# TUI-NICR/EMSANet

Hardware: AMD Instinct MI355X
Metric: images/sec (640x480 RGB-D, bs=32/GPU) fwd+bwd (higher is better)
Workload: dtype f32; 1 GPU; BASELINE.json configs[1]: full EMSANet RGB-D (resnet34-NBt1D x2, SE-add fusion, PPM, semantic+instance+orientation+scene heads), 640x480, bs=32/GPU, f32, train mode (BN batch stats, Dropout2d), step = fwd + bwd (fixed output cotangents) + grad all-reduce + SGD-nesterov update at lr 0 (fixed weights) replayed from a hipGraph; global_batch=32, parallelism=dp1, weights=random init (deterministic), mode=train-hipgraph

## Files before the change

### emsanet_amd/_lib.py

```python
import ctypes
import os
from ctypes import POINTER, Structure, c_char_p, c_float, c_int, c_int8, c_int32, c_int64, c_uint32, c_void_p

LIB_PATH = os.environ.get('EMSA_LIB') or os.path.join(
    os.path.dirname(os.path.abspath(__file__)), 'lib', 'libemsanet_hip.so')


class EmsaPackJob(Structure):
    _fields_ = [('src', c_void_p), ('dst0', c_void_p), ('dst1', c_void_p), ('cout', c_int32),
                ('cin', c_int32), ('kh', c_int32), ('kw', c_int32), ('kind', c_int32),
                ('first_block', c_int32), ('cout_total', c_int32), ('cout_off', c_int32),
                ('cin_total', c_int32), ('cin_off', c_int32)]


PACK_GEMM = 0
PACK_WINO = 1
PACK_GEMM_16 = {1: 2, 2: 3}
PACK_COPY = 4
PACK_FRAG_16 = {1: 5, 2: 6}
PACK_WINO2D = 7


class EmsaDropoutJob(Structure):
    _fields_ = [('offset', c_int64), ('c', c_int32), ('layer_id', c_uint32), ('p', c_float),
# ... 12 lines not shown
        ('in_img_stride', c_int64), ('in_row_stride', c_int64),
        ('in_px_stride', c_int32), ('ld_out', c_int32),
        ('out_pix_img', c_int32), ('out_pix_row', c_int32), ('out_pix_px', c_int32),
        ('out_pix_off', c_int32),
    ]


class EmsaTargetScale(Structure):
    _fields_ = [('scale', c_int32), ('sigma', c_int32), ('semantic', c_void_p), ('center', c_void_p),
                ('offset', c_void_p), ('foreground', c_void_p), ('orientation', c_void_p),
                ('orientation_foreground', c_void_p)]


class EmsaExportJob(Structure):
    _fields_ = [('src0', c_void_p), ('src1', c_void_p), ('depth', c_void_p), ('lut', c_void_p),
                ('dst', c_void_p), ('divisor', c_int64), ('max_depth', ctypes.c_double),
                ('kind', c_int32), ('src0_dtype', c_int32), ('src1_dtype', c_int32),
                ('depth_dtype', c_int32), ('lut_size', c_int32), ('add', c_int32), ('h', c_int32),
                ('w', c_int32)]


class EmsaNormalScale(Structure):
    _fields_ = [('scale', c_int32), ('reserved', c_int32), ('out', c_void_p)]


_P = c_void_p
_GP = POINTER(EmsaConvGeom)
_TP = POINTER(EmsaTargetScale)

SIGNATURES = {
    'emsa_arch': (c_char_p, []),
    'emsa_version': (c_int, []),
    'emsa_set_batch_invariant': (c_int, [c_int]),
    'emsa_conv_igemm': (c_int, [_GP, _P, _P, _P, _P, _P, _P, _P, _P, c_int32, _P, c_int32, c_int32, _P]),
    'emsa_conv_stats_rows': (c_int, [_GP]),
    'emsa_conv1d_wino_supported': (c_int, [_GP]),
    'emsa_conv1d_wino_stats_rows': (c_int, [_GP]),
    'emsa_conv_relu_bits_words': (c_int64, [c_int64, c_int32]),
    'emsa_conv1d_wino_bnb': (c_int, [_GP, _P, _P, _P, _P, c_int32, _P, c_int32, _P, _P, _P, _P, _P,
                                     c_int32, _P]),
    'emsa_conv_igemm_bnb_t': (c_int, [c_int32, _GP, _P, _P, _P, _P, c_int32, _P, c_int32, _P, _P, _P, _P,
                                      _P, c_int32, _P]),
    'emsa_bn_bwd_apply_rows_t': (c_int, [c_int32, _P, _P, _P, _P, _P, _P, c_int32, c_int32, c_int64,
                                         c_int32, c_int32, _P, _P, _P, _P]),
    'emsa_conv1d_wino': (c_int, [_GP, _P, _P, _P, _P, _P, _P, _P, _P, c_int32, _P, c_int32, c_int32, _P,
                                 _P, _P]),
    'emsa_memset_async': (c_int, [_P, c_int32, c_int64, _P]),
    'emsa_graph_count_nodes': (c_int, [_P, POINTER(c_int32), POINTER(c_int32), POINTER(c_int32)]),
    'emsa_graph_replace_memsets': (c_int, [_P, POINTER(c_int32)]),
    'emsa_dropout2d_mask_batch': (c_int, [_P, _P, c_int32, c_int32, c_int32, c_uint32, _P, _P]),
    'emsa_to_nhwc_t': (c_int, [c_int32, _P, _P, c_int32, c_int32, c_int32, c_int32, c_int64, c_int64,
                               c_int64, c_int64, _P]),
    'emsa_conv1d_wino_set_spec': (c_int, [c_int32]),
    'emsa_conv1d_wino_spec_launches': (c_int, []),
    'emsa_conv1d_wino_resmask_supported': (c_int, [_GP, c_int32]),
    'emsa_conv1d_wino_resmask': (c_int, [_GP, _P, _P, _P, _P, c_int32, _P, _P]),
    'emsa_bn_act_fwd_wbits': (c_int, [_P, _P, _P, _P, _P, _P, c_int32, c_int64, c_int32, c_int32, _P, _P]),
    'emsa_bn_act_fwd_raff': (c_int, [_P] * 8 + [c_int32, c_int64, c_int32, c_int32, _P, c_int32, _P]),
    'emsa_bn_bwd_reduce_wbits': (c_int, [_P, _P, _P, _P, _P, _P, c_int32, c_int64, c_int32, _P, _P]),
    'emsa_bn_bwd_apply_wbits': (c_int, [_P] * 8 + [c_int32, c_int32, c_int64, c_int32, c_int32] + [_P] * 5),
    'emsa_conv1d_wino_inbn': (c_int, [_GP, _P, _P, _P, _P, _P, _P, _P, c_int32, _P, _P]),
    'emsa_conv_wgrad_inbn': (c_int, [_GP, _P, _P, _P, _P, _P, _P, _P, _P]),
    'emsa_conv_wgrad_inbn_t': (c_int, [c_int32, _GP, _P, _P, _P, _P, _P, _P, _P, _P]),
    'emsa_conv_wgrad_multi_inbn_t': (c_int, [c_int32, c_int32, _GP, POINTER(c_void_p), POINTER(c_void_p),
                                             POINTER(c_void_p), POINTER(c_void_p), _P,
                                             POINTER(c_void_p), POINTER(c_void_p), _P]),
    'emsa_conv1d_rs_inbn_t': (c_int, [c_int32, _GP, _P, _P, _P, _P, _P, _P, _P, c_int32, _P]),
    'emsa_bn_bwd_reduce_aff_t': (c_int, [c_int32, _P, _P, _P, _P, _P, _P, c_int32, c_int64, c_int32, _P, _P]),
    'emsa_bn_bwd_apply_aff_t': (c_int, [c_int32, _P, _P, _P, _P, _P, _P, _P, _P, c_int32, c_int32, c_int64,
                                        c_int32, _P, _P, _P, _P]),
    'emsa_conv_wgrad_multi_ws_bytes': (c_int64, [c_int32, c_int32, _GP]),
    'emsa_conv_wgrad_multi_t': (c_int, [c_int32, c_int32, _GP, POINTER(c_void_p), POINTER(c_void_p),
                                        POINTER(c_void_p), POINTER(c_void_p), _P, _P]),
    'emsa_pack_wino': (c_int, [_P, _P, _P, c_int32, c_int32, c_int32, _P]),
    'emsa_pack_batch': (c_int, [_P, c_int32, c_int32, _P]),
    'emsa_conv_wino2d_supported': (c_int, [_GP]),
    'emsa_conv_wino2d_stats_rows': (c_int, [_GP]),
    'emsa_conv_wino2d': (c_int, [_GP, _P, _P, _P, _P, _P, _P, _P, _P, c_int32, _P, c_int32, c_int32, _P]),
    'emsa_conv_wgrad_wino2d_supported': (c_int, [c_int32, _GP]),
    'emsa_conv_wgrad_wino2d_ws_bytes': (c_int64, [c_int32, _GP]),
    'emsa_conv_wgrad_wino2d_split_steps': (c_int, [c_int32, _GP]),
    'emsa_conv_wgrad_wino2d': (c_int, [c_int32, _GP, _P, _P, _P, _P, _P, c_int32, _P]),
    'emsa_pack_wino2d': (c_int, [_P, _P, _P, c_int32, c_int32, _P]),
    'emsa_pack_wino2d_packed': (c_int, [_P, _P, c_int32, c_int32, c_int32, _P]),
    'emsa_pack_wino_packed': (c_int, [_P, _P, c_int32, c_int32, c_int32, c_int32, _P]),
    'emsa_conv_wgrad_ws_bytes': (c_int64, [_GP]),
    'emsa_conv_wgrad': (c_int, [_GP, _P, _P, _P, _P, _P, _P]),
    'emsa_pack_weight_fwd': (c_int, [_P, _P] + [c_int32] * 8 + [_P]),
    'emsa_pack_weight_dgrad': (c_int, [_P, _P] + [c_int32] * 8 + [_P]),
    'emsa_unpack_wgrad': (c_int, [_P, _P] + [c_int32] * 8 + [_P]),
    'emsa_pack_weight_pair': (c_int, [_P, _P, _P] + [c_int32] * 4 + [_P]),
    'emsa_stem_pack_input': (c_int, [_P, _P, c_int32, c_int32, c_int32, c_int32, _P]),
    'emsa_stem_pack_weight': (c_int, [_P, _P, c_int32, c_int32, _P]),
    'emsa_stem_pack_input_rows_t': (c_int, [c_int32, _P, _P, c_int32, c_int32, c_int32, _P]),
    'emsa_stem_pack_weight_rows_t': (c_int, [c_int32, _P, _P, c_int32, _P]),
    'emsa_stem_unpack_wgrad_rows': (c_int, [_P, _P, c_int32, _P]),
    'emsa_stem_unpack_wgrad': (c_int, [_P, _P, c_int32, c_int32, _P]),
    'emsa_bn_finalize': (c_int, [_P, c_int32, c_int32, c_int64, _P, _P, c_float, c_float,
                                 _P, _P, _P, _P, _P, _P, _P, _P]),
    'emsa_bn_finalize_ws_bytes': (c_int, [c_int32]),
    'emsa_bn_fold': (c_int, [_P, _P, _P, _P, c_float, c_int32, _P, _P, _P, _P]),
    'emsa_relu_mask_words': (c_int64, [c_int64]),
    'emsa_bn_act_fwd': (c_int, [_P, _P, _P, _P, _P, _P, c_int32, c_int64, c_int32, c_int32, _P,
                                _P]),
    'emsa_bn_bwd_reduce': (c_int, [_P, _P, _P, _P, _P, _P, _P, c_int32, c_int64, c_int32, c_int32,
                                   _P, _P]),
# ... 216 lines not shown
```

### emsanet_amd/csrc/common.h

```cpp
#pragma once
#include <hip/hip_runtime.h>
#include <stdint.h>

#include "emsanet_hip.h"

typedef float f32x16 __attribute__((ext_vector_type(16)));
typedef float f32x4 __attribute__((ext_vector_type(4)));

#define EMSA_WAVE 64
#define EMSA_NXCD 8

static inline int emsa_launch_status() {
  return hipGetLastError() == hipSuccess ? EMSA_OK : EMSA_E_LAUNCH;
}

__device__ __forceinline__ int emsa_xcd_remap(int bid, int nwg) {
  const int q = nwg / EMSA_NXCD, r = nwg % EMSA_NXCD;
  const int xcd = bid % EMSA_NXCD, idx = bid / EMSA_NXCD;
  const int base = xcd < r ? xcd * (q + 1) : r * (q + 1) + (xcd - r) * q;
  return base + idx;
}

__device__ __forceinline__ float4 emsa_ld4(const float* p) {
  return *reinterpret_cast<const float4*>(p);
}
__device__ __forceinline__ void emsa_st4(float* p, float4 v) {
  *reinterpret_cast<float4*>(p) = v;
}
__device__ __forceinline__ float4 emsa_zero4() { return make_float4(0.f, 0.f, 0.f, 0.f); }

__host__ __device__ __forceinline__ size_t emsa_wino2d_at(int comp, int n, int k, int n_ch, int k_ch) {
  return ((((size_t)comp * ((k_ch + 7) >> 3) + (k >> 3)) * n_ch + n) << 3) + (k & 7);
}
__host__ __device__ __forceinline__ int emsa_wino2d_flip(int comp) {
  const int i = comp >> 2, j = comp & 3;
  return (i == 0 ? 3 : i == 3 ? 0 : i) * 4 + (j == 0 ? 3 : j == 3 ? 0 : j);
}
__device__ __forceinline__ void emsa_wino2d_u(const float g[9], float u[16]) {
  float t[3][4];
#pragma unroll
  for (int r = 0; r < 3; ++r) {
    const float s = 0.5f * (g[r * 3] + g[r * 3 + 2]), h = 0.5f * g[r * 3 + 1];
    t[r][0] = g[r * 3]; t[r][1] = s + h; t[r][2] = s - h; t[r][3] = g[r * 3 + 2];
  }
#pragma unroll
  for (int j = 0; j < 4; ++j) {
    const float s = 0.5f * (t[0][j] + t[2][j]), h = 0.5f * t[1][j];
    u[j] = t[0][j]; u[4 + j] = s + h; u[8 + j] = s - h; u[12 + j] = t[2][j];
  }
}

typedef __bf16 emsa_bf16;
typedef _Float16 emsa_f16;
typedef __bf16 emsa_bf16x4 __attribute__((ext_vector_type(4)));
typedef _Float16 emsa_f16x4 __attribute__((ext_vector_type(4)));
typedef float emsa_f32x4v __attribute__((ext_vector_type(4)));

__device__ __forceinline__ float4 emsa_ld4(const emsa_bf16* p) {
  const emsa_f32x4v v = __builtin_convertvector(*reinterpret_cast<const emsa_bf16x4*>(p), emsa_f32x4v);
  return make_float4(v.x, v.y, v.z, v.w);
}
__device__ __forceinline__ float4 emsa_ld4(const emsa_f16* p) {
  const emsa_f32x4v v = __builtin_convertvector(*reinterpret_cast<const emsa_f16x4*>(p), emsa_f32x4v);
  return make_float4(v.x, v.y, v.z, v.w);
}
__device__ __forceinline__ void emsa_st4(emsa_bf16* p, float4 v) {
  const emsa_f32x4v f = {v.x, v.y, v.z, v.w};
  *reinterpret_cast<emsa_bf16x4*>(p) = __builtin_convertvector(f, emsa_bf16x4);
}
__device__ __forceinline__ void emsa_st4(emsa_f16* p, float4 v) {
  const emsa_f32x4v f = {v.x, v.y, v.z, v.w};
  *reinterpret_cast<emsa_f16x4*>(p) = __builtin_convertvector(f, emsa_f16x4);
}
__device__ __forceinline__ float emsa_ld1(const float* p) { return *p; }
__device__ __forceinline__ float emsa_ld1(const emsa_bf16* p) { return (float)*p; }
__device__ __forceinline__ float emsa_ld1(const emsa_f16* p) { return (float)*p; }
__device__ __forceinline__ void emsa_st1(float* p, float v) { *p = v; }
__device__ __forceinline__ void emsa_st1(emsa_bf16* p, float v) { *p = (emsa_bf16)v; }
__device__ __forceinline__ void emsa_st1(emsa_f16* p, float v) { *p = (emsa_f16)v; }

#define EMSA_DISPATCH_DTYPE(dtype, T, ...)                              \
  switch (dtype) {                                                      \
    case EMSA_DT_F32: { using T = float; __VA_ARGS__; } break;          \
    case EMSA_DT_BF16: { using T = emsa_bf16; __VA_ARGS__; } break;     \
    case EMSA_DT_F16: { using T = emsa_f16; __VA_ARGS__; } break;       \
    default: return EMSA_E_ARG;                                         \
  }

static __global__ void emsa_zero_kernel(uint32_t* __restrict__ p, long n_words) {
  for (long i = blockIdx.x * (long)blockDim.x + threadIdx.x; i < n_words;
       i += (long)gridDim.x * blockDim.x)
    p[i] = 0u;
}
static inline void emsa_zero_async(void* p, size_t bytes, hipStream_t st) {
  const long words = (long)(bytes / 4);
  long blocks = (words + 255) / 256;
  if (blocks > 1024) blocks = 1024;
  if (blocks < 1) blocks = 1;
  hipLaunchKernelGGL(emsa_zero_kernel, dim3((int)blocks), dim3(256), 0, st, (uint32_t*)p, words);
}

__device__ __forceinline__ int emsa_nearest_src(int o, int in, int out) {
// ... 14 lines not shown
```

### emsanet_amd/csrc/conv_wino.hip

```cpp
#include <atomic>
#include <cstdlib>
#include <type_traits>

#include "common.h"
#include "prof.h"

namespace {

constexpr int kWK = 16;
constexpr int kWLD = kWK;
constexpr int kPairs = 32;

typedef unsigned int u32x4w __attribute__((ext_vector_type(4)));
typedef __bf16 wbf16x8 __attribute__((ext_vector_type(8)));
constexpr uint32_t kOOBw = 0x80000000u;
__device__ __forceinline__ __amdgpu_buffer_rsrc_t wrsrc(const void* p, uint32_t bytes) {
  return __builtin_amdgcn_make_buffer_rsrc(const_cast<void*>(p), 0, (int)bytes, 0x00020000);
}
__device__ __forceinline__ float4 wbuf_ld4(__amdgpu_buffer_rsrc_t r, uint32_t off) {
  return __builtin_bit_cast(float4, __builtin_amdgcn_raw_buffer_load_b128(r, (int)off, 0, 0));
}
__device__ __forceinline__ float4 wbuf_ld4s(__amdgpu_buffer_rsrc_t r, uint32_t voff, uint32_t soff) {
  return __builtin_bit_cast(float4,
                            __builtin_amdgcn_raw_buffer_load_b128(r, (int)voff, (int)soff, 0));
}
typedef float wf32x2 __attribute__((ext_vector_type(2)));
typedef unsigned int wu32x2 __attribute__((ext_vector_type(2)));

struct WinoArgs {
  const float* in;
  const float* u;
  float* out;
  const float* bias;
  float* stats;
  const float* scale;
  const float* shift;
  const float* residual;
  const float* mask_src;
  const uint64_t* mask_bits;
  int mask_res;
  uint64_t* relu_bits;
  const float* bnb_mean;
  const float* bnb_invstd;
  float* bnb_out;
  int bnb_rows_alloc;
  const float* in_scale;
  const float* in_shift;
  int ld_out, ld_res, ld_mask, act;
  int L, PL, A, MP;
  int k_ch, n_ch;
  int R, c_in, ksteps_c;
  int in_simg, in_sa, in_sb;
  int px_simg, px_sa, px_sb;
  int tiles_m, tiles_n, ksteps;
  uint32_t in_bytes, u_bytes;
  uint32_t mul_pl, sh_pl, mul_a, sh_a;
};

__device__ __forceinline__ int wswz(int row, int c4) {
  return row * kWLD + (c4 ^ (((row >> 2) & 3) << 2));
}

__device__ __forceinline__ uint32_t wdiv(uint32_t n, uint32_t mul, uint32_t sh) {
  return (__umulhi(n, mul) + n) >> sh;
}

#ifndef EMSA_WINO_ST_AUX
#define EMSA_WINO_ST_AUX 0
#endif
#ifndef EMSA_WINO_PRIO
#define EMSA_WINO_PRIO 2
#endif
enum : int {
  kOBias = 1, kORelu = 2, kORBits = 4, kOStats = 8, kOMBits = 16, kORes = 32, kOMRes = 64
};
template <int kWN, bool BF16 = false, bool BNB = false, bool INBN = false, int OPT = -1>
__global__ __launch_bounds__(256, kWN == 64 ? (BNB ? 4 : 5) : 6) void conv1d_wino_kernel(const WinoArgs p) {
  constexpr bool SPEC = OPT >= 0;
  static_assert(!SPEC || (kWN == 64 && !BF16), "specialised epilogues: fp32, 64-channel tiles");
  const bool f_bias = SPEC ? (OPT & kOBias) != 0 : p.bias != nullptr;
  const bool f_relu = SPEC ? (OPT & kORelu) != 0 : p.act == EMSA_ACT_RELU;
  const bool f_rbits = SPEC ? (OPT & kORBits) != 0 : p.relu_bits != nullptr;
  const bool f_stats = SPEC ? (OPT & kOStats) != 0 : p.stats != nullptr;
  const bool f_mbits = SPEC ? (OPT & kOMBits) != 0 : p.mask_bits != nullptr;
  const bool f_res = SPEC ? (OPT & kORes) != 0 : p.residual != nullptr;
  const bool f_mres = SPEC ? (OPT & kOMRes) != 0 : p.mask_res != 0;
  const bool f_scale = SPEC ? BNB : p.scale != nullptr;
  const bool f_msrc = SPEC ? BNB : p.mask_src != nullptr;
  constexpr int NT = kWN / 32;
  constexpr int NC4 = kWN / 4;
  constexpr int RG = 256 / NC4;
  constexpr int PXI = 64 / RG;
  constexpr int BLD = 4 * kWN * 4 / 256;
  extern __shared__ __attribute__((aligned(16))) float smem[];
  float* const As = smem;
  float* const Bs = smem + 4 * kPairs * kWLD;
  float* const Ts = Bs + 4 * kWN * kWLD;

  const int tid = threadIdx.x, lane = tid & 63, wave = __builtin_amdgcn_readfirstlane(tid >> 6);
  const int l31 = lane & 31, lh = lane >> 5;
  const int wg = emsa_xcd_remap(blockIdx.x, gridDim.x);
  const int nt = wg % p.tiles_n, mt = wg / p.tiles_n;
  const int q0 = mt * kPairs, n0 = nt * kWN;
  const __amdgpu_buffer_rsrc_t rs_in = wrsrc(p.in, p.in_bytes);
  const __amdgpu_buffer_rsrc_t rs_u = wrsrc(p.u, p.u_bytes);

  const int c4 = (tid & 3) * 4;
  uint32_t a_base[2], a_voff[2], b_voff[BLD];
  int a_line[2];
  auto setup_a = [&](int mtile) {
#pragma unroll
    for (int j = 0; j < 2; ++j) {
      const int rowid = (tid >> 2) + 64 * j;
      const int rr = rowid >> 5, pr = rowid & 31;
      const int q = mtile * kPairs + pr;
      uint32_t off = kOOBw;
      int al = 0;
      if (q < p.MP) {
        const int line = (int)wdiv((uint32_t)q, p.mul_pl, p.sh_pl);
        const int pp = q - line * p.PL;
        const int img = (int)wdiv((uint32_t)line, p.mul_a, p.sh_a);
        const int a = line - img * p.A;
        const int b = 2 * pp - 1 + rr;
        if (b >= 0 && b < p.L)
          off = (uint32_t)(img * p.in_simg + a * p.in_sa + b * p.in_sb + c4) * 4u;
        al = a;
      }
      a_base[j] = off;
      a_line[j] = al;
    }
  };
  if constexpr (SPEC) {
    const int rr0 = tid >> 7, q = q0 + ((tid >> 2) & 31);
    a_voff[0] = a_voff[1] = kOOBw;
    if (q < p.MP) {
      const int line = (int)wdiv((uint32_t)q, p.mul_pl, p.sh_pl);
      const int pp = q - line * p.PL;
      const int img = (int)wdiv((uint32_t)line, p.mul_a, p.sh_a);
      const int a = line - img * p.A;
      const int base = img * p.in_simg + a * p.in_sa + c4;
#pragma unroll
      for (int j = 0; j < 2; ++j) {
        const int b = 2 * pp - 1 + rr0 + 2 * j;
        if (b >= 0 && b < p.L) a_voff[j] = (uint32_t)(base + b * p.in_sb) * 4u;
      }
    }
  } else {
    setup_a(mt);
  }
#pragma unroll
  for (int j = 0; j < BLD; ++j) {
    const int rowid = (tid >> 2) + 64 * j;
    const int comp = rowid / kWN, n = n0 + (rowid % kWN);
    b_voff[j] = n < p.n_ch ? (uint32_t)((comp * p.n_ch + n) * p.k_ch + c4) * 4u : kOOBw;
  }
  auto set_row = [&](int r) {
    const int dr = !SPEC && p.R == 3 ? r - 1 : 0;
#pragma unroll
    for (int j = 0; j < 2; ++j) {
      const int al = a_line[j] + dr;
      const bool ok = !(a_base[j] & kOOBw) && al >= 0 && al < p.A;
      a_voff[j] = ok ? a_base[j] + (uint32_t)(dr * p.in_sa * 4) : kOOBw;
    }
  };
  const uint32_t last_oob = (p.ksteps_c - 1) * kWK + c4 < p.c_in ? 0u : kOOBw;
  float4 ra[2], rb[BLD];
  auto load_regs = [&](int s) {
    if constexpr (SPEC) {
      const uint32_t so = (uint32_t)(s * kWK) * 4u;
#pragma unroll
      for (int j = 0; j < 2; ++j) ra[j] = wbuf_ld4s(rs_in, a_voff[j], so);
#pragma unroll
      for (int j = 0; j < BLD; ++j) rb[j] = wbuf_ld4s(rs_u, b_voff[j], so);
      return;
    }
    const int r = s >= 2 * p.ksteps_c ? 2 : (s >= p.ksteps_c ? 1 : 0);
    const int ch = (s - r * p.ksteps_c) * kWK;
    if (ch == 0) set_row(r);
    const uint32_t sa = (uint32_t)ch * 4u, sb = (uint32_t)(r * p.c_in + ch) * 4u;
    const uint32_t pm = ch + kWK > p.c_in ? 0xFFFFFFFFu : 0u;
#pragma unroll
    for (int j = 0; j < 2; ++j) ra[j] = wbuf_ld4s(rs_in, a_voff[j] | (last_oob & pm), sa);
#pragma unroll
    for (int j = 0; j < BLD; ++j) rb[j] = wbuf_ld4s(rs_u, b_voff[j] | (last_oob & pm), sb);
  };
  auto store_lds = [&](int s) {
    if constexpr (INBN) {
      const int kt = p.ksteps_c * kWK;
      const float4 sc = emsa_ld4(Ts + s * kWK + c4), sh = emsa_ld4(Ts + kt + s * kWK + c4);
#pragma unroll
      for (int j = 0; j < 2; ++j) {
        const float cap = __uint_as_float(0x7F800000u & ~(uint32_t)((int32_t)a_voff[j] >> 31));
        const wf32x2 lo = __builtin_elementwise_fma(wf32x2{ra[j].x, ra[j].y}, wf32x2{sc.x, sc.y},
                                                    wf32x2{sh.x, sh.y});
        const wf32x2 hi = __builtin_elementwise_fma(wf32x2{ra[j].z, ra[j].w}, wf32x2{sc.z, sc.w},
                                                    wf32x2{sh.z, sh.w});
        ra[j] = make_float4(__builtin_amdgcn_fmed3f(lo.x, 0.f, cap),
                            __builtin_amdgcn_fmed3f(lo.y, 0.f, cap),
                            __builtin_amdgcn_fmed3f(hi.x, 0.f, cap),
                            __builtin_amdgcn_fmed3f(hi.y, 0.f, cap));
      }
    }
#pragma unroll
    for (int j = 0; j < 2; ++j) emsa_st4(As + wswz((tid >> 2) + 64 * j, c4), ra[j]);
#pragma unroll
    for (int j = 0; j < BLD; ++j) emsa_st4(Bs + wswz((tid >> 2) + 64 * j, c4), rb[j]);
  };

  const int ra_ = wave == 0 ? 0 : wave == 2 ? 2 : 1;
  const int rb_ = wave == 2 ? 1 : wave == 3 ? 3 : 2;
  const float sg = wave == 1 ? 1.f : -1.f;

  load_regs(0);
  f32x16 acc[NT];
  if constexpr (!SPEC) {
#pragma unroll
    for (int t = 0; t < NT; ++t)
#pragma unroll
      for (int r = 0; r < 16; ++r) acc[t][r] = 0.f;
  }

  if constexpr (INBN) {
    const int kt = p.ksteps_c * kWK;
    for (int i = tid; i < kt; i += 256) {
      Ts[i] = i < p.c_in ? p.in_scale[i] : 0.f;
      Ts[kt + i] = i < p.c_in ? p.in_shift[i] : 0.f;
    }
    __syncthreads();
  }
  store_lds(0);
  __syncthreads();
  auto kstep = [&](int s, auto first_c) {
// ... 284 lines not shown
        __builtin_amdgcn_raw_buffer_store_b128(__builtin_bit_cast(u32x4w, v), rs_out, (int)off, 0,
                                               EMSA_WINO_ST_AUX);
      }
      if constexpr (SPEC) {
        if (f_rbits) {
          const uint64_t b0 = __builtin_amdgcn_ballot_w64(v.x > 0.f);
          const uint64_t b1 = __builtin_amdgcn_ballot_w64(v.y > 0.f);
          const uint64_t b2 = __builtin_amdgcn_ballot_w64(v.z > 0.f);
          const uint64_t b3 = __builtin_amdgcn_ballot_w64(v.w > 0.f);
          const int sh16 = (lane >> 4) * 16;
          const uint32_t t0 = (uint32_t)(b0 >> sh16), t1 = (uint32_t)(b1 >> sh16);
          const uint32_t t2 = (uint32_t)(b2 >> sh16), t3 = (uint32_t)(b3 >> sh16);
          const wu32x2 word = {__builtin_amdgcn_perm(t1, t0, 0x05040100u),
                               __builtin_amdgcn_perm(t3, t2, 0x05040100u)};
          const uint32_t boff = (col4 == 0 && opix[k] != kNoPix)
                                    ? (opix[k] * (uint32_t)p.tiles_n + (uint32_t)nt) * 8u : kOOBw;
          __builtin_amdgcn_raw_buffer_store_b64(word, wrsrc(p.relu_bits, kOOBw), (int)boff, 0, 0);
        }
      } else if constexpr (kWN == 64) {
        if (f_rbits) {
          const uint64_t b0 = __ballot(live && v.x > 0.f), b1 = __ballot(live && v.y > 0.f);
          const uint64_t b2 = __ballot(live && v.z > 0.f), b3 = __ballot(live && v.w > 0.f);
          const int sh16 = (lane >> 4) * 16;
          if (col4 == 0 && opix[k] != kNoPix)
            p.relu_bits[(size_t)opix[k] * p.tiles_n + nt] =
                ((b0 >> sh16) & 0xFFFFull) | (((b1 >> sh16) & 0xFFFFull) << 16) |
                (((b2 >> sh16) & 0xFFFFull) << 32) | (((b3 >> sh16) & 0xFFFFull) << 48);
        }
      }
    }
    if constexpr (bnb) {
      __syncthreads();
      float* red0 = smem;
      float* red1 = smem + RG * kWN;
      emsa_st4(red0 + rgi * kWN + col4 * 4, make_float4(b0lo.x, b0lo.y, b0hi.x, b0hi.y));
      emsa_st4(red1 + rgi * kWN + col4 * 4, make_float4(b1lo.x, b1lo.y, b1hi.x, b1hi.y));
      __syncthreads();
      if (tid < kWN && n0 + tid < p.n_ch) {
        float a0 = 0.f, a1 = 0.f;
#pragma unroll
        for (int g2 = 0; g2 < RG; ++g2) {
          a0 += red0[g2 * kWN + tid];
          a1 += red1[g2 * kWN + tid];
        }
        p.bnb_out[((size_t)0 * p.bnb_rows_alloc + mt) * p.n_ch + n0 + tid] = a0;
        p.bnb_out[((size_t)1 * p.bnb_rows_alloc + mt) * p.n_ch + n0 + tid] =
            a1 * p.bnb_invstd[n0 + tid];
      }
    }
  }
}

__global__ void pack_wino_kernel(const float* __restrict__ w, float* __restrict__ u,
                                 float* __restrict__ ud, int cout, int cin, int R) {
  const int total = cout * cin * R;
  for (int i = blockIdx.x * blockDim.x + threadIdx.x; i < total; i += gridDim.x * blockDim.x) {
    const int r = i % R, ci = (i / R) % cin, co = i / (R * cin);
    const float* g = w + (size_t)i * 3;
    const float g0 = g[0], g1 = g[1], g2 = g[2];
    const float s = 0.5f * (g0 + g2), h = 0.5f * g1;
    if (u) {
      const size_t NK = (size_t)cout * R * cin, o = ((size_t)co * R + r) * cin + ci;
      u[0 * NK + o] = g0;
      u[1 * NK + o] = s + h;
      u[2 * NK + o] = s - h;
      u[3 * NK + o] = g2;
    }
    if (ud) {
      const size_t NK = (size_t)cin * R * cout, o = ((size_t)ci * R + (R - 1 - r)) * cout + co;
      ud[0 * NK + o] = g2;
      ud[1 * NK + o] = s + h;
      ud[2 * NK + o] = s - h;
      ud[3 * NK + o] = g0;
    }
  }
}

__global__ void pack_wino_packed_kernel(const float* __restrict__ wp, float* __restrict__ u, int n,
                                        int k, int R, int flip) {
  const int total = n * k * R;
  const size_t NK = (size_t)total, plane = (size_t)n * k;
  for (int i = blockIdx.x * blockDim.x + threadIdx.x; i < total; i += gridDim.x * blockDim.x) {
    const int kk = i % k, r = (i / k) % R, nn = i / (k * R);
    const int rs = flip ? R - 1 - r : r;
    const float* g = wp + (size_t)rs * 3 * plane + (size_t)nn * k + kk;
    float g0 = g[0], g1 = g[plane], g2 = g[2 * plane];
    if (flip) { const float t = g0; g0 = g2; g2 = t; }
    const float s = 0.5f * (g0 + g2), h = 0.5f * g1;
    const size_t o = ((size_t)nn * R + r) * k + kk;
    u[0 * NK + o] = g0;
    u[1 * NK + o] = s + h;
    u[2 * NK + o] = s - h;
    u[3 * NK + o] = g2;
  }
}


__device__ __forceinline__ void pack_store(float* base, int r, int n, int k, int nT, int kT,
                                           float v, int kind) {
  size_t idx = ((size_t)r * nT + n) * kT + k;
  if (kind == 5 || kind == 6)
    idx = ((((size_t)r * (nT >> 5) + (n >> 5)) * (kT >> 4) + (k >> 4)) * 64 + (n & 31) +
           32 * ((k & 15) >> 3)) * 8 + (k & 7);
  if (kind == 2 || kind == 5)
    reinterpret_cast<emsa_bf16*>(base)[idx] = (emsa_bf16)v;
  else if (kind == 3 || kind == 6)
    reinterpret_cast<emsa_f16*>(base)[idx] = (emsa_f16)v;
  else
    base[idx] = v;
}
__global__ __launch_bounds__(256) void pack_batch_kernel(const EmsaPackJob* __restrict__ jobs,
                                                         int n_jobs) {
  __shared__ float tr[4][32][33];
  int lo = 0, hi = n_jobs - 1;
  while (lo < hi) {
    const int mid = (lo + hi + 1) >> 1;
    if (jobs[mid].first_block <= (int)blockIdx.x) lo = mid; else hi = mid - 1;
  }
  const EmsaPackJob jb = jobs[lo];
  const int nblk = (lo + 1 < n_jobs ? jobs[lo + 1].first_block : (int)gridDim.x) - jb.first_block;
  const int cout = jb.cout, cin = jb.cin;
  const int coT = jb.cout_total > 0 ? jb.cout_total : cout, ciT = jb.cin_total > 0 ? jb.cin_total : cin;
  const int coO = jb.cout_off, ciO = jb.cin_off;
  if (jb.kind == 4) {
    for (int i = (blockIdx.x - jb.first_block) * 256 + threadIdx.x; i < cout; i += nblk * 256)
      jb.dst0[coO + i] = jb.src[i];
    return;
  }
  const int tx = threadIdx.x & 31, ty = threadIdx.x >> 5;
  const int tco = (cout + 31) / 32, tci = (cin + 31) / 32;
  const bool wino = jb.kind == 1;
  const int taps = jb.kh * jb.kw;
  const bool wino2 = jb.kind == 7;
  const int R = wino ? ((jb.kh == 3 && jb.kw == 3) ? 3 : 1) : (wino2 ? 1 : taps);
  const int n_tiles = tco * tci * R;
  for (int tile = blockIdx.x - jb.first_block; tile < n_tiles; tile += nblk) {
    const int r = tile % R, t2 = tile / R, ci0 = (t2 % tci) * 32, co0 = (t2 / tci) * 32;
    if (wino2) {
      float v2[4][16];
#pragma unroll
      for (int k = 0; k < 4; ++k) {
        const int co = co0 + ty + 8 * k, ci = ci0 + tx;
        const bool ok = co < cout && ci < cin;
        float g[9];
#pragma unroll
        for (int t = 0; t < 9; ++t) g[t] = ok ? jb.src[((size_t)co * cin + ci) * 9 + t] : 0.f;
        emsa_wino2d_u(g, v2[k]);
        if (ok && jb.dst0) {
#pragma unroll
          for (int c = 0; c < 16; ++c)
            jb.dst0[emsa_wino2d_at(c, co + coO, ci + ciO, coT, ciT)] = v2[k][c];
        }
      }
      if (jb.dst1) {
#pragma unroll
        for (int i = 0; i < 4; ++i) {
          __syncthreads();
#pragma unroll
          for (int k = 0; k < 4; ++k)
#pragma unroll
            for (int j = 0; j < 4; ++j) tr[j][ty + 8 * k][tx] = v2[k][i * 4 + j];
          __syncthreads();
#pragma unroll
          for (int k = 0; k < 4; ++k) {
            const int ci = ci0 + ty + 8 * k, co = co0 + tx;
            if (ci < cin && co < cout) {
#pragma unroll
              for (int j = 0; j < 4; ++j)
                jb.dst1[emsa_wino2d_at(emsa_wino2d_flip(i * 4 + j), ci + ciO, co + coO, ciT, coT)] =
                    tr[j][tx][ty + 8 * k];
            }
          }
        }
      }
      continue;
    }
    float vals[4][4];
#pragma unroll
    for (int k = 0; k < 4; ++k) {
      const int co = co0 + ty + 8 * k, ci = ci0 + tx;
      const bool ok = co < cout && ci < cin;
      if (wino) {
        float g0 = 0.f, g1 = 0.f, g2 = 0.f;
        if (ok) {
          const float* g = jb.src + (((size_t)co * cin + ci) * R + r) * 3;
          g0 = g[0]; g1 = g[1]; g2 = g[2];
        }
        const float sm = 0.5f * (g0 + g2), h = 0.5f * g1;
        vals[k][0] = g0; vals[k][1] = sm + h; vals[k][2] = sm - h; vals[k][3] = g2;
        if (ok && jb.dst0) {
          const size_t NK = (size_t)coT * R * ciT, o = ((size_t)(co + coO) * R + r) * ciT + ci + ciO;
#pragma unroll
          for (int j = 0; j < 4; ++j) jb.dst0[j * NK + o] = vals[k][j];
        }
      } else {
        const float v = ok ? jb.src[((size_t)co * cin + ci) * taps + r] : 0.f;
        vals[k][0] = v;
        if (ok && jb.dst0)
          pack_store(jb.dst0, r, co + coO, ci + ciO, coT, ciT, v, jb.kind);
      }
    }
    if (jb.dst1) {
      const int ncomp = wino ? 4 : 1;
      __syncthreads();
#pragma unroll
      for (int k = 0; k < 4; ++k)
        for (int j = 0; j < ncomp; ++j) tr[j][ty + 8 * k][tx] = vals[k][j];
      __syncthreads();
#pragma unroll
      for (int k = 0; k < 4; ++k) {
        const int ci = ci0 + ty + 8 * k, co = co0 + tx;
        if (ci < cin && co < cout) {
          if (wino) {
            const size_t NK = (size_t)ciT * R * coT,
                         o = ((size_t)(ci + ciO) * R + (R - 1 - r)) * coT + co + coO;
            jb.dst1[0 * NK + o] = tr[3][tx][ty + 8 * k];
            jb.dst1[1 * NK + o] = tr[1][tx][ty + 8 * k];
            jb.dst1[2 * NK + o] = tr[2][tx][ty + 8 * k];
            jb.dst1[3 * NK + o] = tr[0][tx][ty + 8 * k];
          } else {
            pack_store(jb.dst1, r, ci + ciO, co + coO, ciT, coT, tr[0][tx][ty + 8 * k], jb.kind);
          }
        }
      }
    }
  }
}

inline void magic(uint32_t d, uint32_t& mul, uint32_t& sh) {
  uint32_t s = 0;
  while ((1ull << s) < d) ++s;
  sh = s;
  mul = (uint32_t)(((1ull << 32) * ((1ull << s) - d)) / d + 1);
}

}

extern "C" int emsa_pack_wino(const float* w_oihw, float* u, float* u_dgrad, int32_t cout,
                              int32_t cin, int32_t rows, void* stream) {
  if (!w_oihw || (!u && !u_dgrad)) return EMSA_E_ARG;
  if (rows != 1 && rows != 3) return EMSA_E_SHAPE;
  const int total = cout * cin * rows;
  int grid = (total + 255) / 256;
  if (grid > 2048) grid = 2048;
  hipLaunchKernelGGL(pack_wino_kernel, dim3(grid), dim3(256), 0, (hipStream_t)stream, w_oihw, u,
                     u_dgrad, cout, cin, rows);
  return emsa_launch_status();
}

extern "C" int emsa_pack_batch(const EmsaPackJob* jobs_device, int32_t n_jobs,
                               int32_t total_blocks, void* stream) {
  if (!jobs_device) return EMSA_E_ARG;
  if (n_jobs < 1 || total_blocks < n_jobs) return EMSA_E_SHAPE;
  hipLaunchKernelGGL(pack_batch_kernel, dim3(total_blocks), dim3(256), 0, (hipStream_t)stream,
                     jobs_device, n_jobs);
  return emsa_launch_status();
}

extern "C" int emsa_pack_wino_packed(const float* w_packed, float* u, int32_t n_ch, int32_t k_ch,
                                     int32_t rows, int32_t flip, void* stream) {
  if (!w_packed || !u) return EMSA_E_ARG;
  if (rows != 1 && rows != 3) return EMSA_E_SHAPE;
  const int total = n_ch * k_ch * rows;
  int grid = (total + 255) / 256;
  if (grid > 2048) grid = 2048;
  hipLaunchKernelGGL(pack_wino_packed_kernel, dim3(grid), dim3(256), 0, (hipStream_t)stream,
                     w_packed, u, n_ch, k_ch, rows, flip ? 1 : 0);
  return emsa_launch_status();
}

extern "C" int emsa_conv1d_wino_supported(const EmsaConvGeom* g) {
  if (g && (g->out_pix_img || g->out_pix_row || g->out_pix_px || g->out_pix_off)) return 0;
  if (!g) return 0;
  auto tap3 = [](int off, int step) { return (off == -1 || off == 1) && step == -off; };
  const bool aw = g->kh == 1 && g->kw == 3 && g->off_h == 0 && tap3(g->off_w, g->step_w);
  const bool ah = g->kh == 3 && g->kw == 1 && g->off_w == 0 && tap3(g->off_h, g->step_h);
  const bool sq = g->kh == 3 && g->kw == 3 && tap3(g->off_w, g->step_w) &&
                  tap3(g->off_h, g->step_h) && g->off_h == g->off_w;
  if (!(aw || ah || sq)) return 0;
  if (g->mul_h != 1 || g->mul_w != 1 || g->div_h != 1 || g->div_w != 1) return 0;
  if (g->in_h != g->out_h || g->in_w != g->out_w) return 0;
  if ((g->k_ch & 3) || (g->n_ch & 3) || (g->ld_out & 3) || (g->in_px_stride & 3)) return 0;
  if ((long)g->n_img * g->in_img_stride >= (1L << 29)) return 0;
  return 1;
}

extern "C" int64_t emsa_conv_relu_bits_words(int64_t pixels, int32_t n_ch) {
  return pixels * ((n_ch + 63) / 64);
}

extern "C" int emsa_conv1d_wino_stats_rows(const EmsaConvGeom* g) {
  if (!emsa_conv1d_wino_supported(g)) return EMSA_E_SHAPE;
  const bool aw = g->kw == 3;
  const int L = aw ? g->out_w : g->out_h, A = aw ? g->out_h : g->out_w;
  const long mp = (long)g->n_img * A * ((L + 1) / 2);
  return (int)((mp + kPairs - 1) / kPairs);
}

static int wino_wn() {
  static const int forced_wn = [] {
    const char* e = getenv("EMSA_WINO_WN");
    return e ? atoi(e) : 0;
  }();
  return forced_wn == 32 || forced_wn == 64 ? forced_wn : 64;
}

static std::atomic<int> g_wino_spec{[] {
  const char* e = getenv("EMSA_WINO_SPEC");
  return e && e[0] == '0' ? 0 : 1;
}()};
static std::atomic<int> g_wino_spec_launches{0};
extern "C" int emsa_conv1d_wino_set_spec(int32_t on) {
  return g_wino_spec.exchange(on ? 1 : 0, std::memory_order_relaxed);
}
extern "C" int emsa_conv1d_wino_spec_launches(void) {
  return g_wino_spec_launches.load(std::memory_order_relaxed);
}

constexpr int wino_spec_key(bool bnb, bool inbn, int opt) {
  return opt | (bnb ? 0x100 : 0) | (inbn ? 0x200 : 0);
}
static int wino_spec_opt(const WinoArgs& a, int wn, bool bf16) {
  if (!g_wino_spec.load(std::memory_order_relaxed) || wn != 64 || bf16 || a.R != 1 || (a.c_in % kWK)) return -1;
  const bool bnb = a.bnb_out != nullptr;
  if (!bnb && (a.scale || a.mask_src)) return -1;
  if (a.act != EMSA_ACT_NONE && a.act != EMSA_ACT_RELU) return -1;
  const int opt = (a.bias ? kOBias : 0) | (a.act == EMSA_ACT_RELU ? kORelu : 0) |
                  (a.relu_bits ? kORBits : 0) | (a.stats ? kOStats : 0) |
                  (a.mask_bits ? kOMBits : 0) | (a.residual ? kORes : 0) |
                  (a.mask_res ? kOMRes : 0);
  return wino_spec_key(bnb, a.in_scale != nullptr, opt);
}

static int conv1d_wino_impl(const EmsaConvGeom* g, const float* in, const float* u, float* out,
                            const float* bias, float* stats, const float* scale,
                            const float* shift, const float* residual, int32_t ld_res,
                            const float* mask_src, int32_t ld_mask, int32_t act,
                            const uint64_t* mask_bits, uint64_t* relu_bits,
                            const float* bnb_mean, const float* bnb_invstd, float* bnb_out,
                            int32_t bnb_rows_alloc, const float* in_scale, const float* in_shift,
                            void* stream, bool mask_res = false) {
  if (!emsa_conv1d_wino_supported(g)) return EMSA_E_SHAPE;
  if ((in_scale == nullptr) != (in_shift == nullptr)) return EMSA_E_ARG;
  if (!in || !u || !out) return EMSA_E_ARG;
  if ((scale == nullptr) != (shift == nullptr)) return EMSA_E_ARG;
  auto al16 = [](const void* q) { return (((uintptr_t)q) & 15) == 0; };
  if (!al16(out) || !al16(bias) || !al16(scale) || !al16(shift) ||
      (residual && (!al16(residual) || (ld_res & 3))) ||
      (mask_src && (!al16(mask_src) || (ld_mask & 3))))
    return EMSA_E_SHAPE;
  WinoArgs a;
  a.in = in; a.u = u; a.out = out; a.bias = bias; a.stats = stats; a.scale = scale;
  a.shift = shift; a.residual = residual; a.mask_src = mask_src;
  a.mask_bits = mask_bits; a.relu_bits = relu_bits;
  a.mask_res = mask_res ? 1 : 0;
  a.bnb_mean = bnb_mean; a.bnb_invstd = bnb_invstd; a.bnb_out = bnb_out;
  a.bnb_rows_alloc = bnb_rows_alloc;
  a.in_scale = in_scale; a.in_shift = in_shift;
  a.ld_out = g->ld_out; a.ld_res = ld_res; a.ld_mask = ld_mask; a.act = act;
  const bool aw = g->kw == 3;
  const int H = g->out_h, W = g->out_w;
  a.L = aw ? W : H;
  a.A = aw ? H : W;
  a.PL = (a.L + 1) / 2;
  a.MP = g->n_img * a.A * a.PL;
  a.R = g->kh == 3 && g->kw == 3 ? 3 : 1;
  a.c_in = g->k_ch;
  a.k_ch = a.R * g->k_ch; a.n_ch = g->n_ch;
  a.in_simg = (int)g->in_img_stride;
  a.in_sa = aw ? (int)g->in_row_stride : g->in_px_stride;
  a.in_sb = aw ? g->in_px_stride : (int)g->in_row_stride;
  a.px_simg = H * W;
  a.px_sa = aw ? W : 1;
  a.px_sb = aw ? 1 : W;
  const int wn = wino_wn();
  if ((mask_bits || relu_bits) && wn != 64) return EMSA_E_SHAPE;
  if (mask_bits && mask_src) return EMSA_E_ARG;
  if (mask_res && (!mask_bits || !residual || bnb_out || relu_bits || in_scale)) return EMSA_E_ARG;
  a.tiles_m = (a.MP + kPairs - 1) / kPairs;
  a.tiles_n = (g->n_ch + wn - 1) / wn;
  if (bnb_out) {
    if (!mask_src || !scale || !bnb_mean || !bnb_invstd || mask_bits || relu_bits || stats ||
        act != EMSA_ACT_NONE || !al16(bnb_mean) || bnb_rows_alloc < a.tiles_m)
      return EMSA_E_ARG;
  }
  {
    const long px = (long)g->n_img * H * W, lim = 1L << 29;
    if (px * g->ld_out >= lim || (residual && px * ld_res >= lim) ||
        (mask_src && px * ld_mask >= lim) || px * a.tiles_n * 2 >= lim)
      return EMSA_E_SHAPE;
  }
  a.ksteps_c = (g->k_ch + kWK - 1) / kWK;
  a.ksteps = a.R * a.ksteps_c;
  a.in_bytes = (uint32_t)((size_t)g->n_img * g->in_img_stride * sizeof(float));
  a.u_bytes = (uint32_t)((size_t)4 * g->n_ch * a.k_ch * sizeof(float));
  magic((uint32_t)a.PL, a.mul_pl, a.sh_pl);
  magic((uint32_t)a.A, a.mul_a, a.sh_a);
  if (in_scale && (a.R != 1 || bnb_out || wn != 64)) return EMSA_E_SHAPE;
  const size_t lds_main = (size_t)(4 * kPairs + 4 * wn) * kWLD * sizeof(float) +
                          (in_scale ? (size_t)2 * a.ksteps_c * kWK * sizeof(float) : 0);
  const size_t lds_epi = (size_t)4 * (kPairs / 2) * (wn + 4) * sizeof(float);
  const size_t lds = lds_main > lds_epi ? lds_main : lds_epi;
  const double flops = 2.0 * g->n_img * H * W * (double)g->k_ch * g->n_ch * 3.0 * a.R;
  const int ps = emsa_prof_begin(a.R == 3 ? kProfClassWino3x3 : kProfClassWino, flops,
                                 (hipStream_t)stream);
  static const bool bf16 = [] {
    const char* e = getenv("EMSA_BF16_MFMA");
    return e && e[0] == '1';
  }();
  const dim3 grid(a.tiles_m * a.tiles_n);
#define EMSA_WINO_SPEC_CASE(BNB_, INBN_, OPT_)                                                     \
  case wino_spec_key(BNB_, INBN_, OPT_):                                                           \
    hipLaunchKernelGGL((conv1d_wino_kernel<64, false, BNB_, INBN_, OPT_>), grid, dim3(256), lds,   \
                       (hipStream_t)stream, a);                                                    \
    break;
  bool launched = true;
  switch (wino_spec_opt(a, wn, bf16)) {
    EMSA_WINO_SPEC_CASE(false, false, kOBias | kORelu | kORBits)
    EMSA_WINO_SPEC_CASE(false, true, kOBias | kORelu | kORBits)
    EMSA_WINO_SPEC_CASE(false, false, kOBias | kOStats)
    EMSA_WINO_SPEC_CASE(false, false, kOMBits)
// ... 78 lines not shown
```

### include/emsanet_hip.h

```cpp
#ifndef EMSANET_HIP_H
#define EMSANET_HIP_H

#include <stdint.h>

#ifdef __cplusplus
extern "C" {
#endif

#define EMSA_OK 0
#define EMSA_E_SHAPE (-1)
#define EMSA_E_ARG (-2)
#define EMSA_E_LAUNCH (-3)

#define EMSA_ACT_NONE 0
#define EMSA_ACT_RELU 1

#define EMSA_DT_F32 0
#define EMSA_DT_BF16 1
#define EMSA_DT_F16 2

const char* emsa_arch(void);
int emsa_version(void);
int emsa_set_batch_invariant(int on);

typedef struct EmsaConvGeom {
  int32_t n_img;
  int32_t in_h, in_w;
  int32_t out_h, out_w;
  int32_t k_ch;
  int32_t n_ch;
  int32_t kh, kw;
  int32_t mul_h, off_h, step_h, div_h;
  int32_t mul_w, off_w, step_w, div_w;
  int64_t in_img_stride, in_row_stride;
  int32_t in_px_stride;
  int32_t ld_out;
  int32_t out_pix_img, out_pix_row, out_pix_px, out_pix_off;
} EmsaConvGeom;

int emsa_conv_igemm(const EmsaConvGeom* g, const float* in, const float* w, float* out,
                    const float* bias, float* stats, const float* scale, const float* shift,
                    const float* residual, int32_t ld_res, const float* mask_src,
                    int32_t ld_mask, int32_t act, void* stream);
int emsa_conv_stats_rows(const EmsaConvGeom* g);

int64_t emsa_conv_wgrad_ws_bytes(const EmsaConvGeom* g);
int emsa_conv_wgrad(const EmsaConvGeom* g, const float* in, const float* dout, float* dw,
                    float* dbias, float* ws, void* stream);

int emsa_conv1d_wino_supported(const EmsaConvGeom* g);
int emsa_conv1d_wino_stats_rows(const EmsaConvGeom* g);
int64_t emsa_conv_relu_bits_words(int64_t pixels, int32_t n_ch);
int emsa_conv1d_wino(const EmsaConvGeom* g, const float* in, const float* u, float* out,
                     const float* bias, float* stats, const float* scale, const float* shift,
                     const float* residual, int32_t ld_res, const float* mask_src,
                     int32_t ld_mask, int32_t act, const uint64_t* mask_bits,
                     uint64_t* relu_bits, void* stream);
int emsa_conv1d_wino_bnb(const EmsaConvGeom* g, const float* dy, const float* u, float* out,
                         const float* residual, int32_t ld_res, const float* t, int32_t ld_t,
                         const float* bn_scale, const float* bn_shift, const float* bn_mean,
                         const float* bn_invstd, float* partial, int32_t rows_alloc, void* stream);
int emsa_conv1d_wino_set_spec(int32_t on);
int emsa_conv1d_wino_spec_launches(void);
int emsa_conv1d_wino_resmask_supported(const EmsaConvGeom* g, int32_t ld_res);
int emsa_conv1d_wino_resmask(const EmsaConvGeom* g, const float* dy, const float* u, float* out,
                             const float* residual, int32_t ld_res, const uint64_t* res_bits,
                             void* stream);
int emsa_conv1d_wino_inbn(const EmsaConvGeom* g, const float* in, const float* u, float* out,
                          const float* bias, float* stats, const float* in_scale,
                          const float* in_shift, int32_t act, uint64_t* relu_bits, void* stream);
int emsa_conv_wgrad_inbn(const EmsaConvGeom* g, const float* in, const float* dout, float* dw,
                         float* dbias, float* ws, const float* in_scale, const float* in_shift,
                         void* stream);
int emsa_pack_wino(const float* w_oihw, float* u, float* u_dgrad, int32_t cout, int32_t cin,
                   int32_t rows, void* stream);
int emsa_pack_wino_packed(const float* w_packed, float* u, int32_t n_ch, int32_t k_ch,
                          int32_t rows, int32_t flip, void* stream);
int emsa_conv_wino2d_supported(const EmsaConvGeom* g);
int emsa_conv_wino2d_stats_rows(const EmsaConvGeom* g);
int emsa_conv_wino2d(const EmsaConvGeom* g, const float* in, const float* u2, float* out,
                     const float* bias, float* stats, const float* scale, const float* shift,
                     const float* residual, int32_t ld_res, const float* mask_src,
                     int32_t ld_mask, int32_t act, void* stream);
int emsa_conv_wgrad_wino2d_supported(int32_t dtype, const EmsaConvGeom* g);
int64_t emsa_conv_wgrad_wino2d_ws_bytes(int32_t dtype, const EmsaConvGeom* g);
int emsa_conv_wgrad_wino2d_split_steps(int32_t dtype, const EmsaConvGeom* g);
int emsa_conv_wgrad_wino2d(int32_t dtype, const EmsaConvGeom* g, const void* in, const void* dout,
                           float* dw, float* dbias, float* ws, int32_t packed, void* stream);
int emsa_pack_wino2d(const float* w_oihw, float* u, float* u_dgrad, int32_t cout, int32_t cin,
                     void* stream);
int emsa_pack_wino2d_packed(const float* w_packed, float* u, int32_t n_ch, int32_t k_ch,
                            int32_t flip, void* stream);
typedef struct EmsaPackJob {
  const float* src;
  float* dst0;
  float* dst1;
  int32_t cout, cin, kh, kw;
  int32_t kind;
  int32_t first_block;
  int32_t cout_total, cout_off, cin_total, cin_off;
} EmsaPackJob;
int emsa_pack_batch(const EmsaPackJob* jobs_device, int32_t n_jobs, int32_t total_blocks,
                    void* stream);

int emsa_pack_weight_fwd(const float* w_oihw, float* w_packed, int32_t cout, int32_t cin,
                         int32_t kh, int32_t kw, int32_t cout_total, int32_t cout_off,
                         int32_t cin_total, int32_t cin_off,
                         void* stream);
int emsa_pack_weight_dgrad(const float* w_oihw, float* w_packed, int32_t cout, int32_t cin,
                           int32_t kh, int32_t kw, int32_t cout_total, int32_t cout_off,
                           int32_t cin_total, int32_t cin_off,
                           void* stream);
int emsa_pack_weight_pair(const float* w_oihw, float* w_packed_fwd, float* w_packed_dgrad,
                          int32_t cout, int32_t cin, int32_t kh, int32_t kw, void* stream);
int emsa_unpack_wgrad(const float* dw_packed, float* dw_oihw, int32_t cout, int32_t cin,
                      int32_t kh, int32_t kw, int32_t cout_total, int32_t cout_off,
// ... 576 lines not shown
```

Measured before the change: 360.4 images/s.

## Tile Winograd 1D weight layout into 64x16 blocks for contiguous B loads

Adds a tiled storage layout for the transformed Winograd weights U, used when R==1 and the channel counts divide 64 and 16. Each 64(n) x 16(k) x 4-component block becomes one contiguous 16 KiB region. The conv kernel's B-operand offsets and k-step strides, and all three pack kernels, are switched to this layout, which is on by default behind an env/API toggle. The aim is more contiguous, cache-friendly weight fetches per k-step instead of strided rows across the full k_ch. The cost is extra index arithmetic, and every consumer of U must agree on the layout, so any reader not updated here would break.

```diff
diff --git a/emsanet_amd/_lib.py b/emsanet_amd/_lib.py
--- a/emsanet_amd/_lib.py
+++ b/emsanet_amd/_lib.py
@@ -88,6 +88,7 @@
     'emsa_to_nhwc_t': (c_int, [c_int32, _P, _P, c_int32, c_int32, c_int32, c_int32, c_int64, c_int64,
                                c_int64, c_int64, _P]),
     'emsa_conv1d_wino_set_spec': (c_int, [c_int32]),
+    'emsa_wino_set_u_tiled': (c_int, [c_int32]),
     'emsa_conv1d_wino_spec_launches': (c_int, []),
     'emsa_conv1d_wino_resmask_supported': (c_int, [_GP, c_int32]),
     'emsa_conv1d_wino_resmask': (c_int, [_GP, _P, _P, _P, _P, c_int32, _P, _P]),
diff --git a/emsanet_amd/csrc/common.h b/emsanet_amd/csrc/common.h
--- a/emsanet_amd/csrc/common.h
+++ b/emsanet_amd/csrc/common.h
@@ -48,6 +48,14 @@
     const float s = 0.5f * (t[0][j] + t[2][j]), h = 0.5f * t[1][j];
     u[j] = t[0][j]; u[4 + j] = s + h; u[8 + j] = s - h; u[12 + j] = t[2][j];
   }
+}
+
+__host__ __device__ __forceinline__ bool wino_u_tiled(int R, int n_ch, int k_ch) {
+  return R == 1 && n_ch % 64 == 0 && k_ch % 16 == 0;
+}
+__host__ __device__ __forceinline__ size_t wino_u_at(bool tiled, int comp, int n, int k, int n_ch, int K) {
+  return tiled ? ((((size_t)(n >> 6) * (K >> 4) + (k >> 4)) * 4 + comp) << 10) + ((n & 63) << 4) + (k & 15)
+               : ((size_t)comp * n_ch + n) * K + k;
 }
 
 typedef __bf16 emsa_bf16;
diff --git a/emsanet_amd/csrc/conv_wino.hip b/emsanet_amd/csrc/conv_wino.hip
--- a/emsanet_amd/csrc/conv_wino.hip
+++ b/emsanet_amd/csrc/conv_wino.hip
@@ -50,6 +50,7 @@
   int L, PL, A, MP;
   int k_ch, n_ch;
   int R, c_in, ksteps_c;
+  int u_tiled;
   int in_simg, in_sa, in_sb;
   int px_simg, px_sa, px_sb;
   int tiles_m, tiles_n, ksteps;
@@ -148,11 +149,17 @@
   } else {
     setup_a(mt);
   }
+  const bool u_tiled = p.u_tiled != 0;
+  const uint32_t u_step = u_tiled ? 16384u : (uint32_t)kWK * 4u;
+  const uint32_t u_row = u_tiled ? 16u : (uint32_t)p.k_ch;
+  const uint32_t u_comp = u_tiled ? 4096u : (uint32_t)(p.n_ch * p.k_ch) * 4u;
+  const uint32_t u_base = u_tiled ? (uint32_t)((n0 >> 6) * p.ksteps) * 16384u + (uint32_t)(n0 & 63) * 64u
+                                  : (uint32_t)(n0 * p.k_ch) * 4u;
 #pragma unroll
   for (int j = 0; j < BLD; ++j) {
     const int rowid = (tid >> 2) + 64 * j;
-    const int comp = rowid / kWN, n = n0 + (rowid % kWN);
-    b_voff[j] = n < p.n_ch ? (uint32_t)((comp * p.n_ch + n) * p.k_ch + c4) * 4u : kOOBw;
+    const int comp = rowid / kWN, nl = rowid % kWN;
+    b_voff[j] = n0 + nl < p.n_ch ? u_base + comp * u_comp + ((uint32_t)nl * u_row + c4) * 4u : kOOBw;
   }
   auto set_row = [&](int r) {
     const int dr = !SPEC && p.R == 3 ? r - 1 : 0;
@@ -171,13 +178,14 @@
 #pragma unroll
       for (int j = 0; j < 2; ++j) ra[j] = wbuf_ld4s(rs_in, a_voff[j], so);
 #pragma unroll
-      for (int j = 0; j < BLD; ++j) rb[j] = wbuf_ld4s(rs_u, b_voff[j], so);
+      for (int j = 0; j < BLD; ++j) rb[j] = wbuf_ld4s(rs_u, b_voff[j], (uint32_t)s * u_step);
       return;
     }
     const int r = s >= 2 * p.ksteps_c ? 2 : (s >= p.ksteps_c ? 1 : 0);
     const int ch = (s - r * p.ksteps_c) * kWK;
     if (ch == 0) set_row(r);
-    const uint32_t sa = (uint32_t)ch * 4u, sb = (uint32_t)(r * p.c_in + ch) * 4u;
+    const uint32_t sa = (uint32_t)ch * 4u;
+    const uint32_t sb = (uint32_t)(r * p.c_in) * 4u + (uint32_t)(s - r * p.ksteps_c) * u_step;
     const uint32_t pm = ch + kWK > p.c_in ? 0xFFFFFFFFu : 0u;
 #pragma unroll
     for (int j = 0; j < 2; ++j) ra[j] = wbuf_ld4s(rs_in, a_voff[j] | (last_oob & pm), sa);
@@ -568,34 +576,36 @@
 }
 
 __global__ void pack_wino_kernel(const float* __restrict__ w, float* __restrict__ u,
-                                 float* __restrict__ ud, int cout, int cin, int R) {
+                                 float* __restrict__ ud, int cout, int cin, int R, int utile) {
   const int total = cout * cin * R;
+  const bool tu = utile && wino_u_tiled(R, cout, cin), td = utile && wino_u_tiled(R, cin, cout);
   for (int i = blockIdx.x * blockDim.x + threadIdx.x; i < total; i += gridDim.x * blockDim.x) {
     const int r = i % R, ci = (i / R) % cin, co = i / (R * cin);
     const float* g = w + (size_t)i * 3;
     const float g0 = g[0], g1 = g[1], g2 = g[2];
     const float s = 0.5f * (g0 + g2), h = 0.5f * g1;
     if (u) {
-      const size_t NK = (size_t)cout * R * cin, o = ((size_t)co * R + r) * cin + ci;
-      u[0 * NK + o] = g0;
-      u[1 * NK + o] = s + h;
-      u[2 * NK + o] = s - h;
-      u[3 * NK + o] = g2;
+      const int k = r * cin + ci, K = R * cin;
+      u[wino_u_at(tu, 0, co, k, cout, K)] = g0;
+      u[wino_u_at(tu, 1, co, k, cout, K)] = s + h;
+      u[wino_u_at(tu, 2, co, k, cout, K)] = s - h;
+      u[wino_u_at(tu, 3, co, k, cout, K)] = g2;
     }
     if (ud) {
-      const size_t NK = (size_t)cin * R * cout, o = ((size_t)ci * R + (R - 1 - r)) * cout + co;
-      ud[0 * NK + o] = g2;
-      ud[1 * NK + o] = s + h;
-      ud[2 * NK + o] = s - h;
-      ud[3 * NK + o] = g0;
+      const int k = (R - 1 - r) * cout + co, K = R * cout;
+      ud[wino_u_at(td, 0, ci, k, cin, K)] = g2;
+      ud[wino_u_at(td, 1, ci, k, cin, K)] = s + h;
+      ud[wino_u_at(td, 2, ci, k, cin, K)] = s - h;
+      ud[wino_u_at(td, 3, ci, k, cin, K)] = g0;
     }
   }
 }
 
 __global__ void pack_wino_packed_kernel(const float* __restrict__ wp, float* __restrict__ u, int n,
-                                        int k, int R, int flip) {
+                                        int k, int R, int flip, int utile) {
   const int total = n * k * R;
-  const size_t NK = (size_t)total, plane = (size_t)n * k;
+  const size_t plane = (size_t)n * k;
+  const bool tu = utile && wino_u_tiled(R, n, k);
   for (int i = blockIdx.x * blockDim.x + threadIdx.x; i < total; i += gridDim.x * blockDim.x) {
     const int kk = i % k, r = (i / k) % R, nn = i / (k * R);
     const int rs = flip ? R - 1 - r : r;
@@ -603,11 +613,10 @@
     float g0 = g[0], g1 = g[plane], g2 = g[2 * plane];
     if (flip) { const float t = g0; g0 = g2; g2 = t; }
     const float s = 0.5f * (g0 + g2), h = 0.5f * g1;
-    const size_t o = ((size_t)nn * R + r) * k + kk;
-    u[0 * NK + o] = g0;
-    u[1 * NK + o] = s + h;
-    u[2 * NK + o] = s - h;
-    u[3 * NK + o] = g2;
+    u[wino_u_at(tu, 0, nn, r * k + kk, n, R * k)] = g0;
+    u[wino_u_at(tu, 1, nn, r * k + kk, n, R * k)] = s + h;
+    u[wino_u_at(tu, 2, nn, r * k + kk, n, R * k)] = s - h;
+    u[wino_u_at(tu, 3, nn, r * k + kk, n, R * k)] = g2;
   }
 }
 
@@ -626,7 +635,7 @@
     base[idx] = v;
 }
 __global__ __launch_bounds__(256) void pack_batch_kernel(const EmsaPackJob* __restrict__ jobs,
-                                                         int n_jobs) {
+                                                         int n_jobs, int utile) {
   __shared__ float tr[4][32][33];
   int lo = 0, hi = n_jobs - 1;
   while (lo < hi) {
@@ -705,9 +714,10 @@
         const float sm = 0.5f * (g0 + g2), h = 0.5f * g1;
         vals[k][0] = g0; vals[k][1] = sm + h; vals[k][2] = sm - h; vals[k][3] = g2;
         if (ok && jb.dst0) {
-          const size_t NK = (size_t)coT * R * ciT, o = ((size_t)(co + coO) * R + r) * ciT + ci + ciO;
-#pragma unroll
-          for (int j = 0; j < 4; ++j) jb.dst0[j * NK + o] = vals[k][j];
+          const bool tu = utile && wino_u_tiled(R, coT, ciT);
+#pragma unroll
+          for (int j = 0; j < 4; ++j)
+            jb.dst0[wino_u_at(tu, j, co + coO, r * ciT + ci + ciO, coT, R * ciT)] = vals[k][j];
         }
       } else {
         const float v = ok ? jb.src[((size_t)co * cin + ci) * taps + r] : 0.f;
@@ -728,12 +738,12 @@
         const int ci = ci0 + ty + 8 * k, co = co0 + tx;
         if (ci < cin && co < cout) {
           if (wino) {
-            const size_t NK = (size_t)ciT * R * coT,
-                         o = ((size_t)(ci + ciO) * R + (R - 1 - r)) * coT + co + coO;
-            jb.dst1[0 * NK + o] = tr[3][tx][ty + 8 * k];
-            jb.dst1[1 * NK + o] = tr[1][tx][ty + 8 * k];
-            jb.dst1[2 * NK + o] = tr[2][tx][ty + 8 * k];
-            jb.dst1[3 * NK + o] = tr[0][tx][ty + 8 * k];
+            const bool td = utile && wino_u_tiled(R, ciT, coT);
+            const int n = ci + ciO, kk = (R - 1 - r) * coT + co + coO, K = R * coT;
+            jb.dst1[wino_u_at(td, 0, n, kk, ciT, K)] = tr[3][tx][ty + 8 * k];
+            jb.dst1[wino_u_at(td, 1, n, kk, ciT, K)] = tr[1][tx][ty + 8 * k];
+            jb.dst1[wino_u_at(td, 2, n, kk, ciT, K)] = tr[2][tx][ty + 8 * k];
+            jb.dst1[wino_u_at(td, 3, n, kk, ciT, K)] = tr[0][tx][ty + 8 * k];
           } else {
             pack_store(jb.dst1, r, ci + ciO, co + coO, ciT, coT, tr[0][tx][ty + 8 * k], jb.kind);
           }
@@ -750,6 +760,16 @@
   mul = (uint32_t)(((1ull << 32) * ((1ull << s) - d)) / d + 1);
 }
 
+std::atomic<int> g_wino_utile{[] {
+  const char* e = getenv("EMSA_WINO_UTILE");
+  return e && e[0] == '0' ? 0 : 1;
+}()};
+inline int wino_utile_on() { return g_wino_utile.load(std::memory_order_relaxed); }
+
+}
+
+extern "C" int emsa_wino_set_u_tiled(int32_t on) {
+  return g_wino_utile.exchange(on ? 1 : 0, std::memory_order_relaxed);
 }
 
 extern "C" int emsa_pack_wino(const float* w_oihw, float* u, float* u_dgrad, int32_t cout,
@@ -760,7 +780,7 @@
   int grid = (total + 255) / 256;
   if (grid > 2048) grid = 2048;
   hipLaunchKernelGGL(pack_wino_kernel, dim3(grid), dim3(256), 0, (hipStream_t)stream, w_oihw, u,
-                     u_dgrad, cout, cin, rows);
+                     u_dgrad, cout, cin, rows, wino_utile_on());
   return emsa_launch_status();
 }
 
@@ -769,7 +789,7 @@
   if (!jobs_device) return EMSA_E_ARG;
   if (n_jobs < 1 || total_blocks < n_jobs) return EMSA_E_SHAPE;
   hipLaunchKernelGGL(pack_batch_kernel, dim3(total_blocks), dim3(256), 0, (hipStream_t)stream,
-                     jobs_device, n_jobs);
+                     jobs_device, n_jobs, wino_utile_on());
   return emsa_launch_status();
 }
 
@@ -781,7 +801,7 @@
   int grid = (total + 255) / 256;
   if (grid > 2048) grid = 2048;
   hipLaunchKernelGGL(pack_wino_packed_kernel, dim3(grid), dim3(256), 0, (hipStream_t)stream,
-                     w_packed, u, n_ch, k_ch, rows, flip ? 1 : 0);
+                     w_packed, u, n_ch, k_ch, rows, flip ? 1 : 0, wino_utile_on());
   return emsa_launch_status();
 }
 
@@ -883,6 +903,7 @@
   a.R = g->kh == 3 && g->kw == 3 ? 3 : 1;
   a.c_in = g->k_ch;
   a.k_ch = a.R * g->k_ch; a.n_ch = g->n_ch;
+  a.u_tiled = wino_utile_on() && wino_u_tiled(a.R, g->n_ch, g->k_ch) ? 1 : 0;
   a.in_simg = (int)g->in_img_stride;
   a.in_sa = aw ? (int)g->in_row_stride : g->in_px_stride;
   a.in_sb = aw ? g->in_px_stride : (int)g->in_row_stride;
diff --git a/include/emsanet_hip.h b/include/emsanet_hip.h
--- a/include/emsanet_hip.h
+++ b/include/emsanet_hip.h
@@ -62,6 +62,7 @@
                          const float* bn_invstd, float* partial, int32_t rows_alloc, void* stream);
 int emsa_conv1d_wino_set_spec(int32_t on);
 int emsa_conv1d_wino_spec_launches(void);
+int emsa_wino_set_u_tiled(int32_t on);
 int emsa_conv1d_wino_resmask_supported(const EmsaConvGeom* g, int32_t ld_res);
 int emsa_conv1d_wino_resmask(const EmsaConvGeom* g, const float* dy, const float* u, float* out,
                              const float* residual, int32_t ld_res, const uint64_t* res_bits,
```

Result: faster. 366.1 images/s, median of 6 (+1.6%).
